# heitorrapela/HalluciDet

Measured on AMD Instinct MI355X. Metric: images/sec train_hallucidet (640x512, batch 8/GPU), higher is better.
Workload: dtype f16; 1 GPU; train_hallucidet.py fasterrcnn LLVIP batch=8 fp16 on 1xMI355X (BASELINE configs[1]); U-Net resnet34 fwd+bwd, 3 frozen Faster R-CNN R50-FPN passes @300x300 (one batched evaluation of 24 images: trunk, RPN, RoI heads, NMS for all three; the RGB / IR passes' LOSS VALUES, which the reference computes and discards, are not evaluated), loss scaling, value clip 0.5, Adam; global_batch=8, image=1x512x640 IR + 3x512x640 RGB, batch_per_gpu=8, parallelism=dp1

## Files before the change

### hallucidet_amd/_abi.py

```python
import ctypes as C
import os

_HERE = os.path.dirname(os.path.abspath(__file__))
LIB_PATH = os.environ.get("HD_HIP_LIB") or os.path.join(_HERE, "lib", "libhallucidet_hip.so")

ABI_VERSION = 6

HD_ACT_NONE, HD_ACT_RELU, HD_ACT_SIGMOID = 0, 1, 2
HD_OUT_NHWC_F16, HD_OUT_NCHW_F32, HD_OUT_NHWC_F32 = 0, 1, 2

c_i32 = C.c_int32
c_i64 = C.c_int64
c_f = C.c_float
c_d = C.c_double
vp = C.c_void_p


class HipLibraryMissing(RuntimeError):
    pass


class HipCallError(RuntimeError):
    pass


class ConvArgs(C.Structure):
    _fields_ = [
        ("x", vp), ("x2", vp), ("w", vp), ("bias", vp), ("res", vp), ("mask", vp), ("y", vp), ("stats", vp),
        ("N", c_i32), ("Hsrc", c_i32), ("Wsrc", c_i32), ("Hin", c_i32), ("Win", c_i32),
        ("C1", c_i32), ("C2", c_i32), ("Ho", c_i32), ("Wo", c_i32), ("Cout", c_i32),
        ("KH", c_i32), ("KW", c_i32), ("stride", c_i32), ("pad", c_i32),
        ("up1", c_i32), ("in_dil", c_i32), ("act", c_i32), ("out_mode", c_i32),
        ("in_scale", vp), ("in_shift", vp), ("in_relu", c_i32), ("out_pool2", c_i32),
        ("bs_y", vp), ("bs_z", vp), ("bs_mean", vp), ("bs_invstd", vp), ("bs_gamma", vp), ("bs_beta", vp), ("bs_relu", c_i32), ("reserved1", c_i32),
        ("y2", vp),
    ]


class WprepDesc(C.Structure):
    _fields_ = [("w_oihw", C.c_void_p), ("w_fwd", C.c_void_p), ("w_dgrad", C.c_void_p)] + \
               [(n, C.c_int32) for n in ("Cout", "Cin", "KH", "KW", "Cin_pad", "Cout_pad")]


class WredDesc(C.Structure):
    _fields_ = [("slab", C.c_void_p), ("dw_oihw", C.c_void_p)] + \
               [(n, C.c_int32) for n in ("nsplit", "Cout_slab", "Cout", "KH", "KW", "Cin", "Cin_real", "accumulate")] + \
               [("scale", C.c_float)] + [(n, C.c_int32) for n in ("mode", "first_block", "reserved")]


class WgradArgs(C.Structure):
    _fields_ = [
        ("x", vp), ("x2", vp), ("dy", vp), ("slab", vp),
        ("N", c_i32), ("Hsrc", c_i32), ("Wsrc", c_i32), ("Hin", c_i32), ("Win", c_i32),
        ("C1", c_i32), ("C2", c_i32), ("Ho", c_i32), ("Wo", c_i32), ("Cout", c_i32),
        ("KH", c_i32), ("KW", c_i32), ("stride", c_i32), ("pad", c_i32), ("up1", c_i32),
        ("nsplit", c_i32),
        ("in_scale", vp), ("in_shift", vp), ("in_relu", c_i32), ("reserved0", c_i32),
        ("dw_oihw", vp), ("dw_scale", c_f), ("reserved1", c_i32),
    ]


PROTOTYPES = {
    "hd_abi_version": (C.c_int, []),
    "hd_last_error": (C.c_char_p, []),
    "hd_arch": (C.c_char_p, []),
    "hd_conv2d": (C.c_int, [C.POINTER(ConvArgs), vp]),
    "hd_conv2d_stats_rows": (C.c_int, [C.POINTER(ConvArgs)]),
    "hd_conv2d_pool2_ok": (C.c_int, [C.POINTER(ConvArgs)]),
    "hd_conv2d_bstat_ok": (C.c_int, [C.POINTER(ConvArgs)]),
    "hd_conv7x7s2_dgrad_thin": (C.c_int, [vp, vp, vp, vp] + [C.c_int] * 5 + [vp]),
    "hd_conv_tune_override": (C.c_int, [C.c_int] * 4),
    "hd_conv_tune_w8": (C.c_int, [C.c_int, C.c_int]),
    "hd_conv_nominal_batch": (C.c_int, [C.c_int]),
    "hd_gemm_w8_mode": (C.c_int, [C.c_int]),
    "hd_wgrad_w8_blocks": (C.c_int, [C.POINTER(WgradArgs)]),
    "hd_wgrad": (C.c_int, [C.POINTER(WgradArgs), vp]),
    "hd_wgrad_multi": (C.c_int, [C.POINTER(WgradArgs), C.c_int, vp]),
    "hd_wgrad_direct_ok": (C.c_int, [C.POINTER(WgradArgs)]),
    "hd_conv2d_wgrad": (C.c_int, [C.POINTER(ConvArgs), C.POINTER(WgradArgs), vp]),
    "hd_conv2d_multi": (C.c_int, [C.POINTER(ConvArgs), C.c_int, vp]),
    "hd_wgrad_tune_override": (C.c_int, [C.c_int]),
    "hd_wgrad_reduce": (C.c_int, [vp, vp] + [C.c_int] * 7 + [c_f, C.c_int, vp]),
    "hd_wgrad_reduce_plan": (C.c_int, [vp, C.c_int]),
    "hd_wgrad_reduce_multi": (C.c_int, [vp, C.c_int, C.c_int, vp]),
    "hd_weight_prep": (C.c_int, [vp, vp, vp, vp] + [C.c_int] * 6 + [vp]),
    "hd_weight_prep_multi": (C.c_int, [vp, C.c_int, C.c_int, vp]),
    "hd_colsum": (C.c_int, [vp, C.c_int, C.c_int, vp, vp, vp]),
    "hd_rowsum": (C.c_int, [vp, C.c_int, C.c_int, vp, C.c_int, vp]),
    "hd_bn_finalize": (C.c_int, [vp, C.c_int, C.c_int, c_d, vp, vp, vp, vp, c_f, c_f, vp, vp, vp, vp, vp]),
    "hd_bn_eval_scale_shift": (C.c_int, [vp, vp, vp, vp, c_f, C.c_int, vp, vp, vp]),
    "hd_bn_apply": (C.c_int, [vp, vp, vp, vp, vp, c_i64, C.c_int, C.c_int, vp]),
    "hd_bn_bwd_reduce": (C.c_int, [vp] * 8 + [C.c_int, c_i64, C.c_int, C.c_int, vp]),
    "hd_bn_bwd_apply": (C.c_int, [vp] * 8 + [C.c_int] + [vp] * 5 + [c_f, C.c_int, c_i64, C.c_int, C.c_int, vp]),
    "hd_maxpool3x3s2": (C.c_int, [vp, vp] + [C.c_int] * 6 + [vp]),
    "hd_maxpool3x3s2_bwd": (C.c_int, [vp, vp, vp] + [C.c_int] * 6 + [vp]),
    "hd_maxpool3x3s2_idx": (C.c_int, [vp, vp, vp] + [C.c_int] * 6 + [vp]),
    "hd_maxpool3x3s2_bwd_idx": (C.c_int, [vp, vp, vp] + [C.c_int] * 6 + [vp]),
    "hd_maxpool3x3s2_bwd_idx_add": (C.c_int, [vp, vp, vp, vp] + [C.c_int] * 6 + [vp]),
    "hd_concat_up_bwd": (C.c_int, [vp, vp, vp] + [C.c_int] * 5 + [vp]),
    "hd_subsample2": (C.c_int, [vp, vp] + [C.c_int] * 6 + [vp]),
    "hd_subsample2_bwd": (C.c_int, [vp, vp] + [C.c_int] * 7 + [vp]),
    "hd_nchw_to_nhwc_resize": (C.c_int, [vp, vp] + [C.c_int] * 7 + [vp]),
    "hd_nchw_to_nhwc_resize_strided": (C.c_int, [vp, c_i64, c_i64, vp] + [C.c_int] * 7 + [vp]),
    "hd_nchw_to_nhwc_resize_bwd": (C.c_int, [vp, vp] + [C.c_int] * 7 + [c_f, vp]),
    "hd_nhwc_to_nchw": (C.c_int, [vp, vp] + [C.c_int] * 5 + [vp]),
    "hd_upsample_add": (C.c_int, [vp, vp, vp] + [C.c_int] * 6 + [vp]),
    "hd_upsample_add_bwd": (C.c_int, [vp, vp] + [C.c_int] * 7 + [vp]),
    "hd_upsample2_bwd": (C.c_int, [vp, vp] + [C.c_int] * 7 + [vp]),
    "hd_add_f16": (C.c_int, [vp, vp, vp, c_i64, vp]),
    "hd_slice_channels": (C.c_int, [vp, vp, c_i64, C.c_int, C.c_int, C.c_int, C.c_int, vp]),
    "hd_sigmoid_bwd_nchw_to_nhwc": (C.c_int, [vp, vp, vp] + [C.c_int] * 5 + [c_f, vp]),
    "hd_relu_bwd": (C.c_int, [vp, vp, vp, c_i64, vp]),
    "hd_f32_to_f16": (C.c_int, [vp, vp, c_i64, c_f, vp]),
    "hd_f16_to_f32": (C.c_int, [vp, vp, c_i64, c_f, vp]),
    "hd_pad_cast_f32_f16": (C.c_int, [vp, vp, C.c_int64, C.c_int, C.c_int, C.c_int64, C.c_int64, vp]),
    "hd_pad_cast_f32_f16_multi": (C.c_int, [vp, vp, vp, vp, vp, vp, vp, C.c_int, vp]),
    "hd_channel_sum_f16": (C.c_int, [vp, c_i64, C.c_int, vp, C.c_int, vp]),
    "hd_scale_store": (C.c_int, [vp, vp, C.c_int, c_f, C.c_int, vp]),
    "hd_nms_sorted_batched": (C.c_int, [vp, vp, C.c_int, C.c_int, c_f, vp, vp, vp]),
    "hd_nms_sorted_batched_topk": (C.c_int, [vp, vp, C.c_int, C.c_int, c_f, vp, vp, C.c_int, vp]),
    "hd_roi_align": (C.c_int, [vp, vp, vp] + [C.c_int] * 7 + [c_f, C.c_int, vp]),
    "hd_roi_align_ml": (C.c_int, [vp, vp, vp, vp, C.c_int, vp, vp, vp] + [C.c_int] * 5 + [vp]),
    "hd_roi_align_ml_bwd": (C.c_int, [vp, vp, vp, vp, vp, vp, vp] + [C.c_int] * 6 + [vp]),
    "hd_roi_align_ml_bwd_gather": (C.c_int, [vp, vp, vp, vp, vp, vp, vp] + [C.c_int] * 7 + [vp]),
    "hd_roi_align_bwd": (C.c_int, [vp, vp, vp] + [C.c_int] * 7 + [c_f, C.c_int, vp]),
    "hd_box_iou": (C.c_int, [vp, C.c_int, vp, C.c_int, vp, vp]),
    "hd_box_iou_batched": (C.c_int, [vp, C.c_int, vp, C.c_int, C.c_int, C.c_int, vp, vp]),
    "hd_rpn_loss": (C.c_int, [vp, vp, vp, vp, vp, vp, C.c_int64, C.c_float, vp, C.c_float, vp, vp, vp]),
    "hd_rpn_loss_bwd": (C.c_int, [vp, vp, vp, vp, vp, vp, C.c_int64, C.c_float, vp, vp, vp, C.c_float, vp, vp, vp]),
    "hd_retinanet_loss": (C.c_int, [vp] * 6 + [C.c_int] * 4 + [C.c_float] * 3 + [vp, vp, vp, vp, vp]),
    "hd_retinanet_loss_bwd": (C.c_int, [vp] * 6 + [C.c_int] * 4 + [C.c_float] * 3 + [vp] * 7),
    "hd_sigmoid_focal_loss": (C.c_int, [vp, vp, C.c_int64, C.c_float, C.c_float, vp, vp, vp]),
    "hd_groupnorm8_relu": (C.c_int, [vp] * 5 + [C.c_int] * 3 + [C.c_float, C.c_int, vp]),
    "hd_groupnorm8_relu_bwd": (C.c_int, [vp] * 6 + [C.c_int] * 4 + [vp]),
    "hd_groupnorm8_param_grad": (C.c_int, [vp] * 6 + [C.c_int] * 4 + [C.c_float, C.c_int, vp]),
    "hd_fcos_match": (C.c_int, [vp] * 3 + [C.c_int] * 5 + [C.c_float, vp, vp]),
    "hd_fcos_loss": (C.c_int, [vp] * 7 + [C.c_int] * 4 + [C.c_float] * 2 + [vp] * 4),
    "hd_fcos_loss_bwd": (C.c_int, [vp] * 7 + [C.c_int] * 4 + [C.c_float] * 2 + [vp] * 6),
    "hd_fastrcnn_loss": (C.c_int, [vp, vp, vp, vp, C.c_int, C.c_int, C.c_float, vp, vp, vp]),
    "hd_fastrcnn_loss_bwd": (C.c_int, [vp, vp, vp, vp, C.c_int, C.c_int, C.c_float, vp, vp, vp, vp, vp]),
    "hd_fastrcnn_loss_masked": (C.c_int, [vp, vp, vp, vp, C.c_int, C.c_int, C.c_float, vp, vp, vp, vp]),
    "hd_fastrcnn_loss_masked_bwd": (C.c_int, [vp, vp, vp, vp, C.c_int, C.c_int, C.c_float, vp, vp, vp, vp, vp, vp]),
    "hd_pixel_loss": (C.c_int, [vp, vp, vp] + [C.c_int] * 5 + [c_f, c_f, C.c_int] + [vp] * 6),
    "hd_augment_u8_ws_bytes": (c_i64, [C.c_int] * 4),
    "hd_augment_u8": (C.c_int, [vp, vp] + [C.c_int] * 4 + [vp, vp, vp]),
    "hd_ir_preprocess_ws_bytes": (c_i64, [C.c_int] * 5),
    "hd_ir_preprocess": (C.c_int, [vp] + [C.c_int] * 4 + [C.POINTER(C.c_int), C.c_int, vp, vp, vp, vp]),
    "hd_map_match": (C.c_int, [vp] * 4 + [C.c_int] * 2 + [vp] * 3 + [C.c_int, vp, C.c_int] + [vp] * 9),
    "hd_map_accumulate": (C.c_int, [vp, vp, vp, c_i64, vp, vp, C.c_int, vp, vp, vp, vp]),
    "hd_sample_pos_neg": (C.c_int, [vp, vp, C.c_int, C.c_int, C.c_int, C.c_int, vp, vp, vp, vp]),
    "hd_roi_postprocess": (C.c_int, [vp, vp, vp, C.c_long, vp, C.c_int, C.c_int, C.c_int, vp] + [C.c_float] * 5 + [vp] * 4),
    "hd_roi_samples_padded": (C.c_int, [vp] * 7 + [C.c_int] * 4 + [vp] * 6),
    "hd_roi_samples_finish": (C.c_int, [vp, C.c_int, vp, vp, vp, vp, vp, C.c_int, C.c_int, vp, vp, vp, vp, vp]),
    "hd_roi_levels": (C.c_int, [vp, C.c_long, C.c_int, C.c_float, C.c_float, C.c_float, C.c_int, C.c_int, vp, vp]),
    "hd_batched_nms_pick": (C.c_int, [vp, vp, vp, vp, C.c_int, C.c_int, C.c_float, C.c_int, vp, vp, vp, vp, vp, vp, vp]),
    "hd_batched_nms_pick_segments": (C.c_int, [vp, vp, vp, C.c_int, C.c_int, vp, C.c_int, C.c_float, C.c_int, vp, vp, vp, vp, vp, vp, vp, vp, vp, vp]),
    "hd_rpn_decode_filter": (C.c_int, [vp, vp, vp, vp, C.c_int, C.c_int, C.c_int, C.c_float, C.c_float, C.c_float, C.c_float, C.c_float, vp, vp, vp, vp]),
    "hd_roi_decode_clip": (C.c_int, [vp, vp, C.c_long, C.c_int, C.c_int, vp, C.c_float, C.c_float, C.c_float, vp, vp]),
# ... 67 lines not shown
```

### hallucidet_amd/csrc/wgrad.hip

```cpp
#include <stdlib.h>

#include "hd_common.h"
#include "hd_lds_dma.h"

namespace {

constexpr int BP = 32;
constexpr int TN = 128;

struct WgP {
  const f16* x;
  const f16* x2;
  const f16* dy;
  float* slab;
  int N, Hsrc, Wsrc, Hin, Win, C1, C2, Cin, Ho, Wo, Cout, KH, KW, stride, pad, up1;
  int M, cin8, nchunks, Ktot, per_split;
  unsigned xbytes, x2bytes, dybytes;
};

typedef __attribute__((address_space(3))) s16x4 lds_s16x4;

__device__ __forceinline__ f16x8 tr_frag(const f16* row0_ptr, int row_stride) {
  s16x4 a = __builtin_amdgcn_ds_read_tr16_b64_v4i16((lds_s16x4*)(row0_ptr));
  s16x4 b = __builtin_amdgcn_ds_read_tr16_b64_v4i16((lds_s16x4*)(row0_ptr + 4 * row_stride));
// ... 419 lines not shown
        float v = 0.f;
        if (ci < d.Cin && co < d.Cout) v = w[((size_t)co * d.Cin + ci) * taps + (taps - 1 - t)];
        wd[i] = (f16)v;
      }
    }
    return;
  }
  constexpr int T = 32;
  __shared__ float tile[T][T * 9 + 1];
  const int co_ext = wd ? (d.Cout_pad > d.Cout ? d.Cout_pad : d.Cout) : d.Cout;
  const int nco = (co_ext + T - 1) / T, nci = (d.Cin_pad + T - 1) / T;
  const int run = T * taps;
  for (int tix = blockIdx.x; tix < nco * nci; tix += gridDim.x) {
    const int co0 = (tix / nci) * T, ci0 = (tix % nci) * T;
    __syncthreads();
    const bool vec_src = (d.Cin % 4) == 0;
    for (int e4 = threadIdx.x; e4 < T * run / 4; e4 += 256) {
      const int r = e4 / (run / 4), j = (e4 - r * (run / 4)) * 4;
      const int co = co0 + r;
      const float* src = w + ((size_t)co * d.Cin + ci0) * taps + j;
      if (vec_src && co < d.Cout && ci0 + (j + 3) / taps < d.Cin) {
        const f32x4 v = *reinterpret_cast<const f32x4*>(src);
        tile[r][j] = v[0]; tile[r][j + 1] = v[1]; tile[r][j + 2] = v[2]; tile[r][j + 3] = v[3];
      } else {
#pragma unroll
        for (int q = 0; q < 4; ++q) tile[r][j + q] = (co < d.Cout && ci0 + (j + q) / taps < d.Cin) ? src[q] : 0.f;
      }
    }
    __syncthreads();
    if (wf) {
      for (int e = threadIdx.x; e < T * taps * (T / 8); e += 256) {
        const int c8 = e % (T / 8), t = (e / (T / 8)) % taps, r = e / ((T / 8) * taps);
        const int co = co0 + r, ci = ci0 + c8 * 8;
        if (co < d.Cout && ci < d.Cin_pad) {
          f16x8 o;
#pragma unroll
          for (int q = 0; q < 8; ++q) o[q] = (f16)tile[r][(c8 * 8 + q) * taps + t];
          *reinterpret_cast<f16x8*>(wf + ((size_t)co * taps + t) * d.Cin_pad + ci) = o;
        }
      }
    }
    if (wd) {
      for (int e = threadIdx.x; e < T * taps * (T / 8); e += 256) {
        const int r8 = e % (T / 8), t = (e / (T / 8)) % taps, ci_l = e / ((T / 8) * taps);
        const int co = co0 + r8 * 8, ci = ci0 + ci_l;
        if (co < d.Cout_pad && ci < d.Cin_pad) {
          f16x8 o;
#pragma unroll
          for (int q = 0; q < 8; ++q) o[q] = (f16)tile[r8 * 8 + q][ci_l * taps + t];
          *reinterpret_cast<f16x8*>(wd + ((size_t)ci * taps + (taps - 1 - t)) * d.Cout_pad + co) = o;
        }
      }
    }
  }
}

}

extern "C" int hd_weight_prep_multi(const hd_wprep_desc* table_dev, int n_layers, int blocks_per_layer, void* stream) {
  HD_CHECK_ARG(table_dev && n_layers > 0 && blocks_per_layer > 0 && blocks_per_layer <= 65535, "hd_weight_prep_multi: bad args");
  hipLaunchKernelGGL(weight_prep_multi_kernel, dim3(blocks_per_layer, n_layers), dim3(256), 0, (hipStream_t)stream, table_dev);
  HD_CHECK_LAUNCH();
  return HD_OK;
}

static int g_wg_tm = -1;
extern "C" int hd_wgrad_tune_override(int tm) {
  HD_CHECK_ARG(tm == -1 || tm == 32 || tm == 64 || tm == 128, "hd_wgrad_tune_override: tm in {32, 64, 128} or -1");
  g_wg_tm = tm;
  return HD_OK;
}

bool hd_wgrad_small_eligible(const hd_wgrad_args* a);
void hd_wgrad_small_launch(const hd_wgrad_args* a, hipStream_t s);
bool hd_wgrad_w8_eligible(const hd_wgrad_args* a);
void hd_wgrad_w8_launch(const hd_wgrad_args* a, hipStream_t s);
extern "C" int hd_wgrad_w8_blocks(const hd_wgrad_args* a) {
  if (!a) return 0;
  static const char* env = getenv("HD_WGRAD_W8");
  if ((env && env[0] == '0') || !hd_wgrad_w8_eligible(a)) return 0;
  return ((a->C1 + a->C2) / 64) * (a->Cout / 64);
}

extern "C" int hd_wgrad_direct_ok(const hd_wgrad_args* a) {
  if (!a || a->nsplit != 1 || a->in_scale) return 0;
  static const char* env8 = getenv("HD_WGRAD_W8");
  static const bool w8_on = !(env8 && env8[0] == '0');
  return (w8_on && g_wg_tm < 0 && !hd_wgrad_small_eligible(a) && hd_wgrad_w8_eligible(a)) ? 1 : 0;
}

bool hd_wgrad_takes_w8(const hd_wgrad_args* a) {
  static const char* env8 = getenv("HD_WGRAD_W8");
  static const bool w8_on = !(env8 && env8[0] == '0');
  if (!a || !a->x || !a->dy || !(a->slab || (a->dw_oihw && a->nsplit == 1)) || a->nsplit < 1 || a->in_scale) return false;
  if (g_wg_tm >= 0 || hd_wgrad_small_eligible(a)) return false;
  return w8_on && hd_wgrad_w8_eligible(a);
}

extern "C" int hd_wgrad(const hd_wgrad_args* a, void* stream) {
  HD_CHECK_ARG(a && a->x && a->dy && (a->slab || a->dw_oihw), "hd_wgrad: null pointer");
  HD_CHECK_ARG(!a->dw_oihw || hd_wgrad_direct_ok(a), "hd_wgrad: dw_oihw (direct output) needs nsplit == 1 and the 8-wave 3x3 kernel (hd_wgrad_direct_ok)");
  HD_CHECK_ARG(a->C1 > 0 && a->C1 % 8 == 0 && a->C2 % 8 == 0 && a->Cout % 8 == 0, "hd_wgrad: channels must be multiples of 8");
  HD_CHECK_ARG((a->C2 == 0) == (a->x2 == nullptr), "hd_wgrad: x2/C2 mismatch");
  HD_CHECK_ARG(a->nsplit >= 1, "hd_wgrad: nsplit");
  HD_CHECK_ARG((a->in_scale == nullptr) == (a->in_shift == nullptr), "hd_wgrad: in_scale / in_shift must be given together");
  {
    static const char* env = getenv("HD_WGRAD_SMALL");
    static const bool small_on = !(env && env[0] == '0');
    if ((small_on || a->in_scale) && g_wg_tm < 0 && hd_wgrad_small_eligible(a)) {
      hd_wgrad_small_launch(a, (hipStream_t)stream);
      HD_CHECK_LAUNCH();
      return HD_OK;
    }
  }
  HD_CHECK_ARG(!a->in_scale, "hd_wgrad: consumer-side BatchNorm (in_scale / in_shift) is implemented by the small-channel 3x3 kernel only "
                             "(3x3 / stride 1 / pad 1, one source, C1 in {16,32}, Cout <= 32)");
  {
    static const char* env8 = getenv("HD_WGRAD_W8");
    static const bool w8_on = !(env8 && env8[0] == '0');
    if (w8_on && g_wg_tm < 0 && hd_wgrad_w8_eligible(a)) {
      hd_wgrad_w8_launch(a, (hipStream_t)stream);
      HD_CHECK_LAUNCH();
      return HD_OK;
    }
  }
  WgP p;
  p.x = (const f16*)a->x; p.x2 = (const f16*)a->x2; p.dy = (const f16*)a->dy; p.slab = a->slab;
  p.N = a->N; p.Hsrc = a->Hsrc; p.Wsrc = a->Wsrc; p.Hin = a->Hin; p.Win = a->Win; p.C1 = a->C1; p.C2 = a->C2;
  p.Cin = a->C1 + a->C2; p.Ho = a->Ho; p.Wo = a->Wo; p.Cout = a->Cout; p.KH = a->KH; p.KW = a->KW;
  p.stride = a->stride; p.pad = a->pad; p.up1 = a->up1;
  p.M = a->N * a->Ho * a->Wo;
  p.cin8 = p.Cin / 8;
  p.nchunks = a->KH * a->KW * p.cin8;
  p.Ktot = a->KH * a->KW * p.Cin;
  int per = hd_cdiv(p.M, a->nsplit);
  per = hd_cdiv(per, BP) * BP;
  p.per_split = per;
  {
    int64_t xb = (int64_t)a->N * a->Hsrc * a->Wsrc * a->C1 * 2, x2b = a->x2 ? (int64_t)a->N * a->Hin * a->Win * a->C2 * 2 : 0;
    int64_t db = (int64_t)p.M * a->Cout * 2;
    HD_CHECK_ARG(xb < 0xFFFFFFF0ll && x2b < 0xFFFFFFF0ll && db < 0xFFFFFFF0ll, "hd_wgrad: tensor larger than 4 GiB (buffer addressing)");
    p.xbytes = (unsigned)xb; p.x2bytes = (unsigned)x2b; p.dybytes = (unsigned)db;
  }
  hipStream_t s = (hipStream_t)stream;
  const int tm = g_wg_tm > 0 ? g_wg_tm : (p.Cout > 64 ? 128 : (p.Cout > 32 ? 64 : 32));
  dim3 grid(hd_cdiv(p.Ktot, TN), hd_cdiv(p.Cout, tm), a->nsplit);
  if (tm == 128) hipLaunchKernelGGL((wgrad_kernel<128, 2, 2>), grid, dim3(256), 0, s, p);
  else if (tm == 64) hipLaunchKernelGGL((wgrad_kernel<64, 2, 2>), grid, dim3(256), 0, s, p);
  else hipLaunchKernelGGL((wgrad_kernel<32, 1, 4>), grid, dim3(256), 0, s, p);
  HD_CHECK_LAUNCH();
  return HD_OK;
}

void hd_wgrad_w8_launch_multi(const hd_wgrad_args* a, int n, hipStream_t s);
extern "C" int hd_wgrad_multi(const hd_wgrad_args* args, int n, void* stream) {
  HD_CHECK_ARG(args && n > 0, "hd_wgrad_multi: bad args");
  static const char* env = getenv("HD_WGRAD_MULTI");
  bool one = !(env && env[0] == '0') && n >= 2 && n <= HD_WGRAD_MULTI_MAX;
  for (int i = 0; i < n; ++i)
    HD_CHECK_ARG(!args[i].dw_oihw || hd_wgrad_direct_ok(args + i), "hd_wgrad_multi: dw_oihw (direct output) needs nsplit == 1 and the 8-wave 3x3 kernel");
  for (int i = 0; one && i < n; ++i) one = hd_wgrad_takes_w8(args + i);
  if (!one) {
    for (int i = 0; i < n; ++i) {
      const int rc = hd_wgrad(args + i, stream);
      if (rc) return rc;
    }
    return HD_OK;
  }
  for (int i = 0; i < n; ++i) {
    const hd_wgrad_args* a = args + i;
    HD_CHECK_ARG(a->C1 > 0 && a->C1 % 8 == 0 && a->C2 % 8 == 0 && a->Cout % 8 == 0 && (a->C2 == 0) == (a->x2 == nullptr) && a->nsplit >= 1,
                 "hd_wgrad_multi: bad entry");
  }
  hd_wgrad_w8_launch_multi(args, n, (hipStream_t)stream);
  HD_CHECK_LAUNCH();
  return HD_OK;
}

static bool red_split_on() {
  static const int on = getenv("HD_WGRAD_REDUCE_SPLIT") ? atoi(getenv("HD_WGRAD_REDUCE_SPLIT")) : 1;
  return on != 0;
}

static bool red_rows_on() {
  static const int on = getenv("HD_WGRAD_REDUCE_ROWS") ? atoi(getenv("HD_WGRAD_REDUCE_ROWS")) : 1;
  return on != 0;
}

extern "C" int hd_wgrad_reduce(const float* slab, float* dw_oihw, int nsplit, int Cout_slab, int Cout, int KH, int KW, int Cin,
                               int Cin_real, float scale, int accumulate, void* stream) {
  HD_CHECK_ARG(slab && dw_oihw && nsplit >= 1 && Cout <= Cout_slab && Cin_real <= Cin, "hd_wgrad_reduce: bad args");
  int64_t total = (int64_t)Cout * Cin * KH * KW / 4;
  int g = (int)((total + 255) / 256);
  if (g > 8192) g = 8192;
  hipStream_t st = (hipStream_t)stream;
  const int mode = red_mode(total, nsplit, red_split_on());
  if (mode >= 4) {
    const int blocks = (int)((total + 63) / 64);
    if (mode == 16)
// ... 64 lines not shown
```

### hallucidet_amd/ops.py

```python
import ctypes as C
import os
import threading

import torch

from . import _abi
from ._abi import ConvArgs, WgradArgs, check, ptr

ACT_NONE, ACT_RELU, ACT_SIGMOID = 0, 1, 2

_tls = threading.local()


def act_dtype():
    return getattr(_tls, "dtype", torch.float16)


class storage:
    def __init__(self, dtype):
        assert dtype in (torch.float16, torch.float32)
        self.dtype = dtype

    def __enter__(self):
        self.prev = getattr(_tls, "dtype", torch.float16)
# ... 31 lines not shown
    assert w.numel() >= Cout * KH * KW * (C1 + C2), "weight tensor too small"
    if in_dil > 1:
        Hin, Win = 0, 0
        assert out_hw is not None
        Ho, Wo = out_hw
    else:
        Hin, Win = (Hs * 2, Ws * 2) if up1 else (Hs, Ws)
        if x2 is not None:
            assert x2.shape[1] == Hin and x2.shape[2] == Win and x2.is_contiguous()
        if out_hw is None:
            Ho, Wo = conv_out_size(Hin, KH, stride, pad), conv_out_size(Win, KW, stride, pad)
        else:
            Ho, Wo = out_hw
    def alloc_y():
        if out is not None:
            return out
        if out_nchw_f32:
            return torch.empty((N, Cout, Ho, Wo), dtype=torch.float32, device=x.device)
        if out_nhwc_f32:
            return torch.empty((N, Ho, Wo, Cout), dtype=torch.float32, device=x.device)
        return torch.empty((N, Ho, Wo, Cout), dtype=x.dtype, device=x.device)

    a = ConvArgs(ptr(x), ptr(x2), ptr(w), ptr(bias), ptr(res), ptr(mask), None, None,
                 N, Hs, Ws, Hin, Win, C1, C2, Ho, Wo, Cout, KH, KW, stride, pad,
                 1 if up1 else 0, in_dil, act, 1 if out_nchw_f32 else (2 if out_nhwc_f32 else 0),
                 ptr(in_scale), ptr(in_shift), 1 if in_relu else 0, 0)
    y, y2 = None, None
    if pool2 is not None:
        pool2["done"] = False
        c_up = int(pool2.get("c_up", Cout))
        if x.dtype == torch.float16 and out is None and not want_stats and bstat is None and Ho % 2 == 0 and Wo % 2 == 0:
            yp = torch.empty((N, Ho // 2, Wo // 2, c_up), dtype=x.dtype, device=x.device)
            y2 = torch.empty((N, Ho, Wo, Cout - c_up), dtype=x.dtype, device=x.device) if Cout > c_up else None
            a.out_pool2, a.y, a.y2 = c_up, ptr(yp), ptr(y2)
            if lib.hd_conv2d_pool2_ok(C.byref(a)) == 1:
                y = yp
                pool2["done"], pool2["skip"] = True, y2
            else:
                a.out_pool2, a.y2, y2 = 0, None, None
                del yp
    if y is None:
        y = alloc_y()
        a.y = ptr(y)
    stats = None
    if bstat is not None:
        bstat["part"] = None
        if x.dtype == torch.float16 and not want_stats and lib.hd_conv2d_bstat_ok(C.byref(a)) == 1:
            rows = lib.hd_conv2d_stats_rows(C.byref(a))
            check(0 if rows > 0 else rows, "hd_conv2d_stats_rows")
            part = torch.empty((rows, 2 * Cout), dtype=torch.float32, device=x.device)
            by, bz = bstat["y"], bstat.get("z")
            assert by.shape == y.shape and by.dtype == y.dtype and by.is_contiguous() and (bz is None or (bz.shape == y.shape and bz.is_contiguous()))
            a.stats, a.bs_y, a.bs_z = ptr(part), ptr(by), ptr(bz)
            a.bs_mean, a.bs_invstd, a.bs_gamma, a.bs_beta = ptr(bstat["mean"]), ptr(bstat["invstd"]), ptr(bstat.get("gamma")), ptr(bstat.get("beta"))
            a.bs_relu = 1 if bstat.get("relu", True) else 0
            bstat["part"] = part
    if want_stats:
        rows = _abi.fn("hd_conv2d_stats_rows", x)(C.byref(a))
        check(0 if rows > 0 else rows, "hd_conv2d_stats_rows")
        stats = torch.empty((rows, 2, Cout), dtype=torch.float32, device=x.device)
        a.stats = ptr(stats)
    if _defer is not None:
        _defer.append((a, (x, x2, w, bias, res, mask, y, y2, stats, in_scale, in_shift, bstat)))
    else:
        check(_abi.fn("hd_conv2d", x)(C.byref(a), _stream()), "hd_conv2d")
    return (y, stats) if want_stats else y


def wgrad(x, dy, KH, KW, *, x2=None, stride=1, pad=0, up1=False, nsplit=None, in_scale=None, in_shift=None, in_relu=True, _defer=None,
          dw=None, dw_scale=1.0):
    _need_cuda(x, dy, x2)
    lib = _abi.load()
    N, Hs, Ws, C1 = x.shape
    C2 = 0 if x2 is None else x2.shape[3]
    _, Ho, Wo, Cout = dy.shape
    Hin, Win = (Hs * 2, Ws * 2) if up1 else (Hs, Ws)
    K = KH * KW * (C1 + C2)
    M = N * Ho * Wo
    if nsplit is None and x.dtype == torch.float32:
        nsplit = pick_nsplit(M, Cout, K)
    if nsplit is None:
        probe = WgradArgs(ptr(x), ptr(x2), ptr(dy), None, N, Hs, Ws, Hin, Win, C1, C2, Ho, Wo, Cout, KH, KW, stride, pad, 1 if up1 else 0, 1)
        blocks8 = lib.hd_wgrad_w8_blocks(C.byref(probe))
        if blocks8 > 0:
            tiles = N * ((Ho + 15) // 16) * ((Wo + 7) // 8)
            nsplit = max(1, min(_WGRAD8_BLOCKS // blocks8, tiles // 4))
            while nsplit > 1 and nsplit * Cout * K * 4 > (64 << 20):
                nsplit //= 2
        elif x2 is not None and up1 and KH == 3 and C1 == 64 and C2 == 64 and Cout <= 32 and stride == 1 and pad == 1:
            nsplit = 256
        else:
            nsplit = pick_nsplit(M, Cout, K)
    direct = False
    if dw is not None and nsplit == 1 and x.dtype == torch.float16:
        probe = WgradArgs(ptr(x), ptr(x2), ptr(dy), None, N, Hs, Ws, Hin, Win, C1, C2, Ho, Wo, Cout, KH, KW, stride, pad, 1 if up1 else 0, 1,
                          ptr(in_scale), ptr(in_shift), 1 if in_relu else 0, 0)
        direct = lib.hd_wgrad_direct_ok(C.byref(probe)) == 1
        if direct:
            assert dw.dtype == torch.float32 and dw.is_contiguous() and dw.numel() == Cout * K
    slab = None if direct else torch.empty((nsplit, Cout, K), dtype=torch.float32, device=x.device)
    a = WgradArgs(ptr(x), ptr(x2), ptr(dy), ptr(slab), N, Hs, Ws, Hin, Win, C1, C2, Ho, Wo, Cout, KH, KW, stride, pad,
                  1 if up1 else 0, nsplit, ptr(in_scale), ptr(in_shift), 1 if in_relu else 0, 0, ptr(dw) if direct else None, float(dw_scale), 0)
    if _defer is not None:
        _defer.append((a, (x, x2, dy, slab, in_scale, in_shift, dw)))
    else:
        check(_abi.fn("hd_wgrad", x)(C.byref(a), _stream()), "hd_wgrad")
    return slab


def stem_dgrad_weights(wf, cin_p=8):
    w = wf.view(64, 7, 7, cin_p).float()
    out = torch.zeros(16, 16, 64, dtype=torch.float32, device=wf.device)
    for a in range(2):
        for b in range(2):
            for di in range(-1, 3):
                for dj in range(-1, 3):
                    kh, kw = a + 3 - 2 * di, b + 3 - 2 * dj
                    if 0 <= kh <= 6 and 0 <= kw <= 6:
                        for c in range(min(3, cin_p)):
                            out[(2 * a + b) * 4 + c, (di + 1) * 4 + dj + 1] = w[:, kh, kw, c]
    return out.view(16, 1024).half().contiguous()


def conv7x7s2_dgrad_thin(dy, w16, in_hw, mask_z=None, out=None):
    _need_cuda(dy, w16, mask_z)
    N, Hl, Wl, C_ = dy.shape
    H, W = in_hw
    assert C_ == 64 and dy.dtype == torch.float16 and dy.is_contiguous() and w16.shape == (16, 1024) and w16.dtype == torch.float16
    assert mask_z is None or (mask_z.shape == dy.shape and mask_z.dtype == dy.dtype and mask_z.is_contiguous())
    if out is not None:
        assert out.shape == (N, H, W, 8) and out.dtype == torch.float16 and out.is_contiguous() and out.device == dy.device
    dx = out if out is not None else torch.empty((N, H, W, 8), dtype=torch.float16, device=dy.device)
    check(_abi.load().hd_conv7x7s2_dgrad_thin(ptr(dy), ptr(mask_z), ptr(w16), ptr(dx), N, Hl, Wl, H, W, _stream()), "hd_conv7x7s2_dgrad_thin")
    return dx


def conv2d_multi(calls):
    if len(calls) == 1 or calls[0][0].dtype == torch.float32:
        return [conv2d(x, w, KH, KW, **kw) for x, w, KH, KW, kw in calls]
    hold, outs = [], []
    for x, w, KH, KW, kw in calls:
        outs.append(conv2d(x, w, KH, KW, _defer=hold, **kw))
    arr = (ConvArgs * len(hold))(*[h[0] for h in hold])
    check(_abi.load().hd_conv2d_multi(arr, len(hold), _stream()), "hd_conv2d_multi")
    return outs


WGRAD_MULTI_MAX = 24


def wgrad_w8_blocks(x, dy, KH, KW, *, x2=None, stride=1, pad=0, up1=False, **_):
    if x.dtype != torch.float16:
        return 0
    N, Hs, Ws, C1 = x.shape
    C2 = 0 if x2 is None else x2.shape[3]
    _, Ho, Wo, Cout = dy.shape
    Hin, Win = (Hs * 2, Ws * 2) if up1 else (Hs, Ws)
    probe = WgradArgs(ptr(x), ptr(x2), ptr(dy), None, N, Hs, Ws, Hin, Win, C1, C2, Ho, Wo, Cout, KH, KW, stride, pad, 1 if up1 else 0, 1)
    return int(_abi.load().hd_wgrad_w8_blocks(C.byref(probe)))


def wgrad_takes_w8(x, dy, KH, KW, **kw):
    return wgrad_w8_blocks(x, dy, KH, KW, **kw) > 0


def wgrad_multi(calls):
    if not calls:
# ... 930 lines not shown
```

### include/hallucidet_hip.h

```cpp
#ifndef HALLUCIDET_HIP_H
#define HALLUCIDET_HIP_H

#include <stdint.h>

#ifdef __cplusplus
extern "C" {
#endif

#define HD_OK 0
#define HD_E_ARG (-1)
#define HD_E_LAUNCH (-2)
#define HD_E_UNSUPPORTED (-3)

#define HD_ACT_NONE 0
#define HD_ACT_RELU 1
#define HD_ACT_SIGMOID 2

#define HD_OUT_NHWC_F16 0
#define HD_OUT_NCHW_F32 1
#define HD_OUT_NHWC_F32 2

int hd_abi_version(void);
const char* hd_last_error(void);
const char* hd_arch(void);

typedef struct hd_conv_args {
  const void* x;
  const void* x2;
  const void* w;
  const float* bias;
  const void* res;
  const void* mask;
  void* y;
  float* stats;
  int32_t N, Hsrc, Wsrc;
  int32_t Hin, Win;
  int32_t C1, C2;
  int32_t Ho, Wo, Cout;
  int32_t KH, KW, stride, pad;
  int32_t up1, in_dil;
  int32_t act, out_mode;
  const float* in_scale;
  const float* in_shift;
  int32_t in_relu;
  int32_t out_pool2;
  const void* bs_y;
  const void* bs_z;
  const float* bs_mean;
  const float* bs_invstd;
  const float* bs_gamma;
  const float* bs_beta;
  int32_t bs_relu, reserved1;
  void* y2;
} hd_conv_args;

int hd_conv2d(const hd_conv_args* a, void* stream);
int hd_conv2d_bstat_ok(const hd_conv_args* a);
int hd_conv2d_pool2_ok(const hd_conv_args* a);
int hd_conv2d_stats_rows(const hd_conv_args* a);
int hd_conv7x7s2_dgrad_thin(const void* dy, const void* mask_z, const void* w16, void* dx, int N, int Hl, int Wl, int H, int W, void* stream);
int hd_conv_tune_override(int bm, int bn, int bk, int deep);
int hd_conv_tune_w8(int cfg, int nslices);
int hd_conv_nominal_batch(int n);
int hd_gemm_w8_mode(int mode);

typedef struct hd_wgrad_args {
  const void* x;
  const void* x2;
  const void* dy;
  float* slab;
  int32_t N, Hsrc, Wsrc, Hin, Win, C1, C2, Ho, Wo, Cout;
  int32_t KH, KW, stride, pad, up1;
  int32_t nsplit;
  const float* in_scale;
  const float* in_shift;
  int32_t in_relu, reserved0;
  float* dw_oihw;
  float dw_scale;
  int32_t reserved1;
} hd_wgrad_args;
int hd_wgrad(const hd_wgrad_args* a, void* stream);
int hd_wgrad_direct_ok(const hd_wgrad_args* a);
#define HD_WGRAD_MULTI_MAX 24
int hd_wgrad_multi(const hd_wgrad_args* args, int n, void* stream);
int hd_wgrad_w8_blocks(const hd_wgrad_args* a);
int hd_wgrad_tune_override(int tm);
int hd_conv2d_multi(const hd_conv_args* args, int n, void* stream);

int hd_conv2d_wgrad(const hd_conv_args* dgrad, const hd_wgrad_args* wgrad, void* stream);

int hd_wgrad_reduce(const float* slab, float* dw_oihw, int nsplit, int Cout_slab, int Cout, int KH, int KW,
                    int Cin, int Cin_real, float scale, int accumulate, void* stream);

#define HD_WRED_MAX 16
typedef struct hd_wred_desc {
  const float* slab;
  float* dw_oihw;
  int32_t nsplit, Cout_slab, Cout, KH, KW, Cin, Cin_real, accumulate;
  float scale;
  int32_t mode, first_block, reserved;
} hd_wred_desc;
int hd_wgrad_reduce_plan(hd_wred_desc* table_host, int n);
int hd_wgrad_reduce_multi(const hd_wred_desc* table_host, int n, int total_blocks, void* stream);

typedef struct hd_wprep_desc {
  const float* w_oihw;
  void* w_fwd;
  void* w_dgrad;
  int32_t Cout, Cin, KH, KW, Cin_pad, Cout_pad;
} hd_wprep_desc;

int hd_weight_prep(const float* w_oihw, const float* out_scale , void* w_fwd ,
                   void* w_dgrad , int Cout, int Cin, int KH, int KW,
                   int Cin_pad, int Cout_pad, void* stream);
int hd_weight_prep_multi(const hd_wprep_desc* table_dev, int n_layers, int blocks_per_layer, void* stream);

int hd_colsum(const float* in, int rows, int W, float* out, float* ws, void* stream);
int hd_rowsum(const float* in, int rows, int W, float* out, int out_rows, void* stream);
int hd_bn_finalize(const float* part, int rows, int C, double count, const float* gamma, const float* beta,
                   float* running_mean, float* running_var, float momentum, float eps, float* mean, float* invstd,
                   float* scale, float* shift, void* stream);
int hd_bn_eval_scale_shift(const float* gamma, const float* beta, const float* running_mean, const float* running_var,
                           float eps, int C, float* scale, float* shift, void* stream);
int hd_bn_apply(const void* y, const void* res, const float* scale, const float* shift, void* z, int64_t n, int C,
                int relu, void* stream);
int hd_bn_bwd_reduce(const void* dz, const void* z, const void* y, const float* mean, const float* invstd,
                     const float* gamma, const float* beta, float* part, int rows, int64_t npix, int C, int relu, void* stream);
int hd_bn_bwd_apply(const void* dz, const void* z, const void* y, const float* mean, const float* invstd,
                    const float* gamma, const float* beta, const float* part, int rows, float* coef_ws, void* dy, void* dres,
                    float* dgamma, float* dbeta, float gscale, int accumulate, int64_t npix, int C, int relu, void* stream);

int hd_maxpool3x3s2(const void* x, void* y, int N, int H, int W, int C, int Ho, int Wo, void* stream);
int hd_maxpool3x3s2_bwd(const void* x, const void* dy, void* dx, int N, int H, int W, int C, int Ho, int Wo, void* stream);
int hd_maxpool3x3s2_idx(const void* x, void* y, void* idx_u8, int N, int H, int W, int C, int Ho, int Wo, void* stream);
int hd_maxpool3x3s2_bwd_idx(const void* idx_u8, const void* dy, void* dx, int N, int H, int W, int C, int Ho, int Wo, void* stream);
int hd_maxpool3x3s2_bwd_idx_add(const void* idx_u8, const void* dy, const void* add, void* dx, int N, int H, int W, int C, int Ho, int Wo,
                                void* stream);
int hd_subsample2(const void* x, void* y, int N, int H, int W, int C, int Ho, int Wo, void* stream);
int hd_subsample2_bwd(const void* dy, void* dx, int N, int H, int W, int C, int Ho, int Wo, int accumulate, void* stream);
int hd_nchw_to_nhwc_resize(const float* x, void* y, int N, int Cr, int H, int W, int Ho, int Wo, int Cp, void* stream);
int hd_nchw_to_nhwc_resize_strided(const float* x, int64_t nstride, int64_t cstride, void* y, int N, int Cr, int H, int W, int Ho,
                                   int Wo, int Cp, void* stream);
int hd_nchw_to_nhwc_resize_bwd(const void* dy, float* dx, int N, int Cr, int H, int W, int Ho, int Wo, int Cp,
                               float gscale, void* stream);
int hd_nhwc_to_nchw(const void* x, float* y, int N, int Cr, int H, int W, int Cp, void* stream);
int hd_upsample_add(const void* a, const void* b, void* y, int N, int H, int W, int C, int Hb, int Wb, void* stream);
int hd_upsample_add_bwd(const void* dy, void* db, int N, int H, int W, int C, int Hb, int Wb, int accumulate, void* stream);
int hd_upsample2_bwd(const void* dy_up, void* dx_low, int N, int Hl, int Wl, int C, int Ctot, int c_off, int accumulate,
                     void* stream);
int hd_concat_up_bwd(const void* dcat, void* dlow, void* dskip, int N, int Hl, int Wl, int Cup, int Cskip, void* stream);
int hd_add_f16(const void* a, const void* b, void* out, int64_t n, void* stream);
int hd_slice_channels(const void* x, void* y, int64_t npix, int Ctot, int c_off, int C, int accumulate, void* stream);
int hd_sigmoid_bwd_nchw_to_nhwc(const float* dy, const float* s, void* dlogit, int N, int Cr, int H, int W, int Cp,
                                float gscale, void* stream);
int hd_relu_bwd(const void* dy, const void* z, void* dx, int64_t n, void* stream);
int hd_f32_to_f16(const float* x, void* y, int64_t n, float scale, void* stream);
int hd_f16_to_f32(const void* x, float* y, int64_t n, float scale, void* stream);
int hd_pad_cast_f32_f16(const float* x, void* y, int64_t P, int C, int Cp, int64_t rows_per_image, int64_t image_stride, void* stream);
int hd_pad_cast_f32_f16_multi(const float* const* x, void* const* y, const int64_t* P, const int* C, const int* Cp,
                              const int64_t* rows_per_image, const int64_t* image_stride, int n, void* stream);
int hd_channel_sum_f16(const void* x, int64_t npix, int C, float* part, int rows, void* stream);
int hd_scale_store(const float* in, float* out, int n, float scale, int accumulate, void* stream);

int hd_nms_sorted_batched(const float* boxes, const int* counts, int B, int nmax, float iou_thr, uint64_t* mask_ws,
                          uint8_t* keep, void* stream);
int hd_nms_sorted_batched_topk(const float* boxes, const int* counts, int B, int nmax, float iou_thr, uint64_t* mask_ws,
                               uint8_t* keep, int max_keep, void* stream);
int hd_roi_align(const void* feat, const float* rois, void* out, int R, int N, int H, int W, int C, int PH, int PW,
// ... 177 lines not shown
```

Measured before the change: 817.7 images/s.

## Add dedicated 7x7 stride-2 stem weight-gradient kernel with MFMA spatial tiling

Adds a specialised wgrad kernel for the ResNet stem conv (7x7, stride 2, pad 3, 8 padded input channels, 64 outputs). Each block covers 8x16 output-pixel tiles and stages an input patch plus dy in double-buffered LDS. It reuses each input row across all kh taps via 32x32x16 MFMAs and writes per-block partial slabs for the existing reduce. It is picked automatically when there are enough tiles, and the split is capped at 256 blocks. The aim is to replace the generic implicit-GEMM path, whose K dimension is small and uses poorly for this layer.

New measurement: 823.8 images/s (median of 6 runs). Within noise of the previous version (+0.7%).

```diff
diff --git a/hallucidet_amd/_abi.py b/hallucidet_amd/_abi.py
--- a/hallucidet_amd/_abi.py
+++ b/hallucidet_amd/_abi.py
@@ -74,6 +74,8 @@
     "hd_conv_nominal_batch": (C.c_int, [C.c_int]),
     "hd_gemm_w8_mode": (C.c_int, [C.c_int]),
     "hd_wgrad_w8_blocks": (C.c_int, [C.POINTER(WgradArgs)]),
+    "hd_wgrad_stem_blocks": (C.c_int, [C.POINTER(WgradArgs)]),
+    "hd_wgrad_stem_mode": (C.c_int, [C.c_int]),
     "hd_wgrad": (C.c_int, [C.POINTER(WgradArgs), vp]),
     "hd_wgrad_multi": (C.c_int, [C.POINTER(WgradArgs), C.c_int, vp]),
     "hd_wgrad_direct_ok": (C.c_int, [C.POINTER(WgradArgs)]),
diff --git a/hallucidet_amd/csrc/wgrad.hip b/hallucidet_amd/csrc/wgrad.hip
--- a/hallucidet_amd/csrc/wgrad.hip
+++ b/hallucidet_amd/csrc/wgrad.hip
@@ -525,6 +525,28 @@
   return ((a->C1 + a->C2) / 64) * (a->Cout / 64);
 }
 
+bool hd_wgrad_stem_eligible(const hd_wgrad_args* a);
+int hd_wgrad_stem_tiles(const hd_wgrad_args* a);
+int hd_wgrad_stem_max_blocks();
+void hd_wgrad_stem_launch(const hd_wgrad_args* a, hipStream_t s);
+static int g_wg_stem = -1;
+extern "C" int hd_wgrad_stem_mode(int mode) {
+  HD_CHECK_ARG(mode == -1 || mode == 0 || mode == 1, "hd_wgrad_stem_mode: mode in {-1, 0, 1}");
+  g_wg_stem = mode;
+  return HD_OK;
+}
+static bool wgrad_takes_stem(const hd_wgrad_args* a) {
+  static const char* env = getenv("HD_WGRAD_STEM");
+  static const bool rule_on = !(env && env[0] == '0');
+  if (g_wg_stem == 0 || g_wg_tm >= 0 || !hd_wgrad_stem_eligible(a)) return false;
+  return g_wg_stem == 1 || (rule_on && hd_wgrad_stem_tiles(a) >= 4 * hd_wgrad_stem_max_blocks());
+}
+extern "C" int hd_wgrad_stem_blocks(const hd_wgrad_args* a) {
+  if (!a || !wgrad_takes_stem(a)) return 0;
+  const int t = hd_wgrad_stem_tiles(a), m = hd_wgrad_stem_max_blocks();
+  return t < m ? t : m;
+}
+
 extern "C" int hd_wgrad_direct_ok(const hd_wgrad_args* a) {
   if (!a || a->nsplit != 1 || a->in_scale) return 0;
   static const char* env8 = getenv("HD_WGRAD_W8");
@@ -558,6 +580,11 @@
   }
   HD_CHECK_ARG(!a->in_scale, "hd_wgrad: consumer-side BatchNorm (in_scale / in_shift) is implemented by the small-channel 3x3 kernel only "
                              "(3x3 / stride 1 / pad 1, one source, C1 in {16,32}, Cout <= 32)");
+  if (wgrad_takes_stem(a)) {
+    hd_wgrad_stem_launch(a, (hipStream_t)stream);
+    HD_CHECK_LAUNCH();
+    return HD_OK;
+  }
   {
     static const char* env8 = getenv("HD_WGRAD_W8");
     static const bool w8_on = !(env8 && env8[0] == '0');
diff --git a/hallucidet_amd/csrc/wgrad7x7s2_stem.hip b/hallucidet_amd/csrc/wgrad7x7s2_stem.hip
--- /dev/null
+++ b/hallucidet_amd/csrc/wgrad7x7s2_stem.hip
@@ -0,0 +1,174 @@
+#include <stdlib.h>
+
+#include "hd_common.h"
+#include "hd_lds_dma.h"
+
+namespace {
+
+typedef __attribute__((address_space(3))) s16x4 lds_s16x4;
+
+constexpr int TH = 8, TW = 16;
+constexpr int PH = 2 * TH + 5, PW = 2 * TW + 5;
+constexpr int NPIX = PH * PW;
+constexpr int XSTAGE = (NPIX + 7) * 8;
+constexpr int DPITCH = 96;
+constexpr int DSTAGE = TH * TW * DPITCH;
+constexpr int NT = 256;
+constexpr int XL = (NPIX + NT - 1) / NT;
+constexpr int DL = TH * TW * 8 / NT;
+constexpr int KTOT = 7 * 7 * 8;
+constexpr int MAXB = 256;
+
+__device__ __forceinline__ f16x8 tr_frag(const f16* row0_ptr, int row_stride) {
+  s16x4 a = __builtin_amdgcn_ds_read_tr16_b64_v4i16((lds_s16x4*)(row0_ptr));
+  s16x4 b = __builtin_amdgcn_ds_read_tr16_b64_v4i16((lds_s16x4*)(row0_ptr + 4 * row_stride));
+  f16x4 fa = __builtin_bit_cast(f16x4, a), fb = __builtin_bit_cast(f16x4, b);
+  f16x8 r = {fa[0], fa[1], fa[2], fa[3], fb[0], fb[1], fb[2], fb[3]};
+  return r;
+}
+
+__global__ __launch_bounds__(NT) void wgrad7x7s2_stem_kernel(const f16* __restrict__ x, const f16* __restrict__ dy, float* __restrict__ slab,
+                                                              int H, int W, int Ho, int Wo, int tiles_total, int tiles_x, int tiles_y,
+                                                              int nwork, unsigned xbytes, unsigned dybytes) {
+  __shared__ __attribute__((aligned(16))) f16 s_x[2][XSTAGE];
+  __shared__ __attribute__((aligned(16))) f16 s_dy[2][DSTAGE];
+  const int tid = threadIdx.x, lane = tid & 63;
+  const int wave = __builtin_amdgcn_readfirstlane(tid >> 6);
+  const int cot = wave & 1, kwh = wave >> 1;
+  float* out = slab + (size_t)blockIdx.x * 64 * KTOT;
+  if ((int)blockIdx.x >= nwork) {
+    for (int i = tid; i < 64 * KTOT / 4; i += NT) reinterpret_cast<f32x4*>(out)[i] = (f32x4){0.f, 0.f, 0.f, 0.f};
+    return;
+  }
+  const int L = hd_xcd_contiguous(blockIdx.x, nwork);
+  const int t_begin = (int)((long long)L * tiles_total / nwork), t_end = (int)((long long)(L + 1) * tiles_total / nwork);
+
+  const __amdgpu_buffer_rsrc_t rxs = __builtin_amdgcn_make_buffer_rsrc(const_cast<f16*>(x), 0, xbytes, 0x00020000);
+  const __amdgpu_buffer_rsrc_t rdy = __builtin_amdgcn_make_buffer_rsrc(const_cast<f16*>(dy), 0, dybytes, 0x00020000);
+
+  int xrel[XL], xpy[XL], xpx[XL];
+#pragma unroll
+  for (int i = 0; i < XL; ++i) {
+    const int pp = tid + i * NT;
+    const int py = pp / PW, px = pp - py * PW;
+    xrel[i] = ((py - 3) * W + (px - 3)) * 16;
+    xpy[i] = pp < NPIX ? py - 3 : -0x40000000;
+    xpx[i] = px - 3;
+  }
+  const int dch = tid & 7, dox = (tid >> 3) & 15, doy = tid >> 7;
+
+  u32x4 rx[2][XL], rd[2][DL];
+  auto gload = [&](int t, u32x4 (&qx)[XL], u32x4 (&qd)[DL]) {
+    const bool live = t < t_end;
+    const int tt = live ? t : t_begin;
+    const int r1 = tt / tiles_x;
+    const int tx = tt - r1 * tiles_x;
+    const int n = r1 / tiles_y;
+    const int ty = r1 - n * tiles_y;
+    const int y0 = ty * (2 * TH), x0 = tx * (2 * TW);
+    const int xbase = ((n * H + y0) * W + x0) * 16;
+#pragma unroll
+    for (int i = 0; i < XL; ++i) {
+      const bool ok = live & ((unsigned)(y0 + xpy[i]) < (unsigned)H) & ((unsigned)(x0 + xpx[i]) < (unsigned)W);
+      qx[i] = __builtin_amdgcn_raw_buffer_load_b128(rxs, ok ? (unsigned)(xbase + xrel[i]) : OOB, 0, 0);
+    }
+#pragma unroll
+    for (int i = 0; i < DL; ++i) {
+      const int oy = ty * TH + doy + 2 * i, ox = tx * TW + dox;
+      const bool ok = live & (oy < Ho) & (ox < Wo);
+      qd[i] = __builtin_amdgcn_raw_buffer_load_b128(rdy, ok ? (unsigned)(((n * Ho + oy) * Wo + ox) * 128 + dch * 16) : OOB, 0, 0);
+    }
+  };
+  auto lstore = [&](int buf, const u32x4 (&qx)[XL], const u32x4 (&qd)[DL]) {
+#pragma unroll
+    for (int i = 0; i < XL; ++i) {
+      const int pp = tid + i * NT;
+      if (pp < NPIX) *reinterpret_cast<u32x4*>(&s_x[buf][pp * 8]) = qx[i];
+    }
+#pragma unroll
+    for (int i = 0; i < DL; ++i) *reinterpret_cast<u32x4*>(&s_dy[buf][((doy + 2 * i) * TW + dox) * DPITCH + dch * 8]) = qd[i];
+  };
+
+  const int li = lane & 15, g = lane >> 4;
+  const int tq = li >> 2, tp = li & 3;
+  const int th = g >> 1, thalf = g & 1;
+  const int krow = 8 * th + tq;
+  const int aoff = krow * DPITCH + cot * 32 + 16 * thalf + 4 * tp;
+  const int boff = (2 * krow + 4 * kwh) * 8 + 16 * thalf + 4 * tp;
+
+  f32x16 acc[7];
+#pragma unroll
+  for (int k = 0; k < 7; ++k)
+#pragma unroll
+    for (int r = 0; r < 16; ++r) acc[k][r] = 0.f;
+
+  auto compute = [&](int buf) {
+    const f16* ap = &s_dy[buf][aoff];
+    const f16* bp = &s_x[buf][boff];
+    f16x8 af[TH];
+#pragma unroll
+    for (int oy = 0; oy < TH; ++oy) af[oy] = tr_frag(ap + oy * TW * DPITCH, DPITCH);
+#pragma unroll
+    for (int r = 0; r < PH; ++r) {
+      const f16x8 bf = tr_frag(bp + r * PW * 8, 16);
+#pragma unroll
+      for (int kh = r & 1; kh < 7; kh += 2) {
+        const int oy = (r - kh) / 2;
+        if (r >= kh && oy < TH) acc[kh] = __builtin_amdgcn_mfma_f32_32x32x16_f16(af[oy], bf, acc[kh], 0, 0, 0);
+      }
+    }
+  };
+
+  gload(t_begin, rx[0], rd[0]);
+  lstore(0, rx[0], rd[0]);
+  gload(t_begin + 1, rx[0], rd[0]);
+  gload(t_begin + 2, rx[1], rd[1]);
+  __syncthreads();
+  for (int t = t_begin; t < t_end; t += 2) {
+    compute(0);
+    lstore(1, rx[0], rd[0]);
+    gload(t + 3, rx[0], rd[0]);
+    __syncthreads();
+    compute(1);
+    lstore(0, rx[1], rd[1]);
+    gload(t + 4, rx[1], rd[1]);
+    __syncthreads();
+  }
+
+  const int j = lane & 31;
+  const int kw = 4 * kwh + (j >> 3);
+  if (kw < 7) {
+#pragma unroll
+    for (int kh = 0; kh < 7; ++kh)
+#pragma unroll
+      for (int r = 0; r < 16; ++r) {
+        const int co = 32 * cot + (r & 3) + 8 * (r >> 2) + 4 * (lane >> 5);
+        out[(size_t)co * KTOT + (kh * 7 + kw) * 8 + (j & 7)] = acc[kh][r];
+      }
+  }
+}
+
+}
+
+bool hd_wgrad_stem_eligible(const hd_wgrad_args* a) {
+  if (a->KH != 7 || a->KW != 7 || a->stride != 2 || a->pad != 3 || a->up1) return false;
+  if (a->C1 != 8 || a->C2 != 0 || a->x2 || a->Cout != 64 || a->in_scale || a->dw_oihw) return false;
+  if (a->N < 1 || a->Hin < 1 || a->Win < 1 || a->Hsrc != a->Hin || a->Wsrc != a->Win) return false;
+  if (a->Ho != (a->Hin + 6 - 7) / 2 + 1 || a->Wo != (a->Win + 6 - 7) / 2 + 1) return false;
+  if ((int64_t)a->N * a->Hin * a->Win * 16 >= (int64_t)1 << 30 || (int64_t)a->N * a->Ho * a->Wo * 128 >= (int64_t)1 << 30) return false;
+  return true;
+}
+
+int hd_wgrad_stem_tiles(const hd_wgrad_args* a) { return a->N * hd_cdiv(a->Ho, TH) * hd_cdiv(a->Wo, TW); }
+
+int hd_wgrad_stem_max_blocks() { return MAXB; }
+
+void hd_wgrad_stem_launch(const hd_wgrad_args* a, hipStream_t s) {
+  const int tiles_x = hd_cdiv(a->Wo, TW), tiles_y = hd_cdiv(a->Ho, TH);
+  const int tiles = a->N * tiles_x * tiles_y;
+  int nwork = a->nsplit < tiles ? a->nsplit : tiles;
+  if (nwork > MAXB) nwork = MAXB;
+  hipLaunchKernelGGL(wgrad7x7s2_stem_kernel, dim3(a->nsplit), dim3(NT), 0, s, (const f16*)a->x, (const f16*)a->dy, a->slab, a->Hin, a->Win,
+                     a->Ho, a->Wo, tiles, tiles_x, tiles_y, nwork, (unsigned)((int64_t)a->N * a->Hin * a->Win * 16),
+                     (unsigned)((int64_t)a->N * a->Ho * a->Wo * 128));
+}
diff --git a/hallucidet_amd/ops.py b/hallucidet_amd/ops.py
--- a/hallucidet_amd/ops.py
+++ b/hallucidet_amd/ops.py
@@ -137,7 +137,10 @@
     if nsplit is None:
         probe = WgradArgs(ptr(x), ptr(x2), ptr(dy), None, N, Hs, Ws, Hin, Win, C1, C2, Ho, Wo, Cout, KH, KW, stride, pad, 1 if up1 else 0, 1)
         blocks8 = lib.hd_wgrad_w8_blocks(C.byref(probe))
-        if blocks8 > 0:
+        stem = lib.hd_wgrad_stem_blocks(C.byref(probe))
+        if stem > 0:
+            nsplit = stem
+        elif blocks8 > 0:
             tiles = N * ((Ho + 15) // 16) * ((Wo + 7) // 8)
             nsplit = max(1, min(_WGRAD8_BLOCKS // blocks8, tiles // 4))
             while nsplit > 1 and nsplit * Cout * K * 4 > (64 << 20):
diff --git a/include/hallucidet_hip.h b/include/hallucidet_hip.h
--- a/include/hallucidet_hip.h
+++ b/include/hallucidet_hip.h
@@ -84,6 +84,8 @@
 #define HD_WGRAD_MULTI_MAX 24
 int hd_wgrad_multi(const hd_wgrad_args* args, int n, void* stream);
 int hd_wgrad_w8_blocks(const hd_wgrad_args* a);
+int hd_wgrad_stem_blocks(const hd_wgrad_args* a);
+int hd_wgrad_stem_mode(int mode);
 int hd_wgrad_tune_override(int tm);
 int hd_conv2d_multi(const hd_conv_args* args, int n, void* stream);
 
```
